# netease-youdao/EmotiVoice

Measured on NVIDIA H100. Metric: mel_frames_per_sec, higher is better.
Workload: dtype fp32 (fp32 storage + accumulate; tensor-core fp32 emulation: 3xTF32 prefix, bf16x3 after it)

## Files before the change

emotivoice_b200/csrc/conv1d_gp.cu:

```cuda
#include "ev_common.cuh"
#include "gp_pipeline.cuh"

namespace ev {
namespace gp {

using namespace gpl;

constexpr int MAX_A = 8;

struct GPlan {
  int BN, mt, kbg, planes;
  int rows_pad;
  int a_plane_bytes, b_plane_bytes, a_stage_bytes, b_stage_bytes;
  int a_stages, b_stages;
  int acc_cols;
  int tiles_m, tiles_n, total_tiles;
  int smem_total;
};

__host__ __device__ inline bool make_gplan(const GpConvParams& p, int mode, int BN, int mt, int kbg, GPlan* o, int span = -1, int kmin = 0, int ng = 1) {
  if (span < 0) span = (p.K - 1) * p.dil;
  if (kmin <= 0) kmin = p.K;
  GPlan q;
  q.planes = mode == 1 ? 2 : 1;
// ... 46 lines not shown
  __syncthreads();

  asm volatile("griddepcontrol.launch_dependents;" ::: "memory");

  const int n_cb = (p.Cin + KB - 1) / KB;
  const int tiles_per_b = pl.tiles_m * pl.tiles_n;
  const int tiles_per_g = p.B * tiles_per_b;

  auto decode = [&](int tile, int& gi, int& b, int& t0, int& n0, int& len) {
    gi = tile / tiles_per_g;
    tile -= gi * tiles_per_g;
    b = tile / tiles_per_b;
    const int r = tile - b * tiles_per_b;
    const int tm = r / pl.tiles_n, tn = r - tm * pl.tiles_n;
    t0 = tm * (BM * MT);
    n0 = tn * BN;
    len = p.lens ? min(p.L, p.lens[b] * p.lens_mul) : p.L;
  };

  if (warp < NCW) {
    asm volatile("griddepcontrol.wait;" ::: "memory");
    const int wg = warp >> 2, wl = warp & 3;
    const int coutR = p.Cout / p.rate;
    const int gout = coutR / CPG;
    const size_t Lout = (size_t)p.L * p.rate;
    const int accm = p.acc;
    const uint32_t a_lbo = (uint32_t)pl.rows_pad * 16u, b_lbo = (uint32_t)BN * 16u;
    const uint64_t a_desc0 = make_desc(0u, X3B ? 2u * a_lbo : a_lbo, 128u), b_desc0 = make_desc(0u, b_lbo, 128u);
    const uint32_t a_k8 = (X3B ? 4u : 2u) * a_lbo;
    const uint32_t a_lo_off = X3B ? a_lbo : (uint32_t)pl.a_plane_bytes;
    float acc[MT][NA];
#pragma unroll
    for (int mt = 0; mt < MT; ++mt)
#pragma unroll
      for (int i = 0; i < NA; ++i) acc[mt][i] = 0.f;
    int a_cnt = 0, b_cnt = 0;
    for (int tile = blockIdx.x; tile < pl.total_tiles; tile += gridDim.x) {
      int gi, b, t0, n0, len;
      decode(tile, gi, b, t0, n0, len);
      if (t0 >= len) continue;
      const GpGroup& G = gs.g[gi];
      const int K = G.K;
      const uint32_t a_tap = (uint32_t)G.dil * 16u;
      OneBehind<MAX_A> rel{ring, lane};
      for (int cb = 0; cb < n_cb; ++cb, ++a_cnt) {
        const int sa = a_cnt % pl.a_stages;
        const int nk8 = min(KB, p.Cin - cb * KB) / (2 * WCPG);
        mbar_wait(ring.a_ready(sa), (a_cnt / pl.a_stages) & 1);
        const uint64_t a_hi0 = desc_advance(a_desc0, smem_u32(a_tiles + sa * pl.a_stage_bytes) + (uint32_t)(wg * 64) * 16u);
        for (int j = 0; j < K; ++j, ++b_cnt) {
          const int sb = b_cnt % pl.b_stages;
          mbar_wait(ring.b_full(sb), (b_cnt / pl.b_stages) & 1);
          const uint64_t b_hi0 = desc_advance(b_desc0, smem_u32(b_tiles + sb * pl.b_stage_bytes));
          tap_chain<MODE, BN, NK8>(acc, desc_advance(a_hi0, (uint32_t)j * a_tap), a_k8, a_lo_off, b_hi0, (uint32_t)pl.b_plane_bytes, cb | j, nk8);
          wgmma_wait<1>();
          rel.step(sb, j == K - 1 ? sa : -1);
        }
      }

      constexpr int EQ = MT == 1 ? 2 : 1;
      const bool has_res = G.res != nullptr;
      const int row0 = t0 + wg * 64 + frag_row(0, lane, wl);
      float2 ebias[EQ];
      pair_t<BF16> eres[EQ][MT][2], eout[EQ][MT][2];
      auto column = [&](int q, int& n) {
        n = n0 + frag_col(4 * q, lane);
        const int phase = n / coutR, co = n - phase * coutR;
        return (((size_t)b * gout + co / CPG) * Lout + phase) * CPG + (co % CPG);
      };
      auto epi_load = [&](int ch) {
#pragma unroll
        for (int q = 0; q < EQ; ++q) {
          int n;
          const size_t ec = column(ch * EQ + q, n);
          if (n - n0 >= BN) continue;
          if (G.bias) ebias[q] = __ldg(reinterpret_cast<const float2*>(G.bias + n));
#pragma unroll
          for (int mt = 0; mt < MT; ++mt)
#pragma unroll
            for (int h = 0; h < 2; ++h) {
              const int row = row0 + mt * BM + 8 * h;
              if (row >= len) continue;
              const size_t e = ec + (size_t)row * p.rate * CPG;
              if (has_res) eres[q][mt][h] = load_pair<BF16>(G.res, e);
              if (accm != EV_ACC_STORE) eout[q][mt][h] = load_pair<BF16>(G.out, e);
            }
        }
      };
      auto epi_store = [&](int ch) {
#pragma unroll
        for (int q = 0; q < EQ; ++q) {
          int n;
          const size_t ec = column(ch * EQ + q, n);
          if (n - n0 >= BN) continue;
#pragma unroll
          for (int mt = 0; mt < MT; ++mt)
#pragma unroll
            for (int h = 0; h < 2; ++h) {
              const int row = row0 + mt * BM + 8 * h;
              if (row >= len) continue;
              const int i = 4 * (ch * EQ + q) + 2 * h;
              float v0 = acc[mt][i], v1 = acc[mt][i + 1];
              if (G.bias) { v0 += ebias[q].x; v1 += ebias[q].y; }
              if (has_res) {
                const float2 r = unpack_pair(eres[q][mt][h]);
                v0 += r.x; v1 += r.y;
              }
              if (accm != EV_ACC_STORE) {
// ... 457 lines not shown
```

emotivoice_b200/csrc/conv1d_tc.cu:

```cuda
#include <cstdio>
#include <cstdlib>

#include "ev_common.cuh"
#include "tc_common.cuh"

namespace ev {

namespace tc {

struct Plan {
  int BN, mt, kbg, planes;
  int rows_pad;
  int a_plane_bytes, b_plane_bytes, a_stage_bytes, b_stage_bytes;
  int a_stages, b_stages;
  int ngroups;
  int ksplit;
  int acc_cols;
  int tiles_m, tiles_n, total_tiles;
  int smem_total;
};

__host__ __device__ inline bool make_plan(const ConvParams& p, int mode, int BN, int mt, int kbg, int min_b_stages, Plan* o, int b_target = 4) {
  Plan q;
  q.planes = (mode == 1 || mode == 3) ? 2 : 1;
// ... 12 lines not shown
  const int budget = 227 * 1024 - 1024;
  const int n_cb = (p.Cin + cpg * q.kbg - 1) / (cpg * q.kbg);
  if (min_b_stages > n_cb * p.K) min_b_stages = n_cb * p.K;
  if (min_b_stages < 2) min_b_stages = 2;
  if (2 * q.a_stage_bytes + min_b_stages * q.b_stage_bytes > budget) return false;
  q.a_stages = 2;
  q.b_stages = 2;
  while (q.b_stages < MAX_B_STAGES && q.b_stages < n_cb * p.K &&
         q.a_stages * q.a_stage_bytes + (q.b_stages + 1) * q.b_stage_bytes <= budget && q.b_stages < b_target) ++q.b_stages;
  while (q.a_stages < MAX_A_STAGES && q.a_stages < n_cb &&
         (q.a_stages + 1) * q.a_stage_bytes + q.b_stages * q.b_stage_bytes <= budget && q.a_stages < 6) ++q.a_stages;
  while (q.b_stages < MAX_B_STAGES && q.b_stages < n_cb * p.K &&
         q.a_stages * q.a_stage_bytes + (q.b_stages + 1) * q.b_stage_bytes <= budget) ++q.b_stages;
  while (q.a_stages < MAX_A_STAGES && q.a_stages < n_cb &&
         (q.a_stages + 1) * q.a_stage_bytes + q.b_stages * q.b_stage_bytes <= budget) ++q.a_stages;
  q.ngroups = q.a_stages >= 6 ? 6 : (q.a_stages >= 3 ? 3 : (q.a_stages >= 2 ? 2 : 1));
  q.tiles_m = (p.L + BM * mt - 1) / (BM * mt);
  q.tiles_n = (p.Cout + q.BN - 1) / q.BN;
  q.ksplit = 1;
  q.total_tiles = p.B * q.tiles_m * q.tiles_n;
  q.smem_total = 1024 + q.a_stages * q.a_stage_bytes + q.b_stages * q.b_stage_bytes;
  *o = q;
  return true;
}

__device__ __forceinline__ void splitk_reduce_store(const ConvParams& p, int S, size_t per, size_t e, int b, int row, int col, int len) {
  float4 o = make_float4(0.f, 0.f, 0.f, 0.f);
  if (row < len) {
    for (int z = 0; z < S; ++z) {
      const float4 v = *reinterpret_cast<const float4*>(p.splitk_ws + (size_t)z * per + e);
      o.x += v.x; o.y += v.y; o.z += v.z; o.w += v.w;
    }
    if (p.bias) {
      const float4 b4 = __ldg(reinterpret_cast<const float4*>(p.bias + (size_t)b * p.bias_bs + col));
      o.x += b4.x; o.y += b4.y; o.z += b4.z; o.w += b4.w;
    }
    if (p.out_act != EV_ACT_NONE) {
      o.x = act_apply(o.x, p.out_act, 0.f); o.y = act_apply(o.y, p.out_act, 0.f);
      o.z = act_apply(o.z, p.out_act, 0.f); o.w = act_apply(o.w, p.out_act, 0.f);
    }
    if (p.res) {
      const float4 r4 = *reinterpret_cast<const float4*>(p.res + e);
      o.x += r4.x; o.y += r4.y; o.z += r4.z; o.w += r4.w;
    }
    if (p.acc != EV_ACC_STORE) {
      const float4 q4 = *reinterpret_cast<const float4*>(p.out + e);
      o.x += q4.x; o.y += q4.y; o.z += q4.z; o.w += q4.w;
      if (p.acc == EV_ACC_ADD_DIV) { o.x /= p.div; o.y /= p.div; o.z /= p.div; o.w /= p.div; }
    }
  }
  *reinterpret_cast<float4*>(p.out + e) = o;
}

template <int MODE, int MT, int KBG>
__global__ void __launch_bounds__(NTHREADS, 1) conv1d_tc_kernel(ConvParams p, Plan pl) {
  constexpr bool SPLIT3 = (MODE == 1);
  constexpr bool X3B = (MODE == 3);
  constexpr bool BF16 = (MODE == 2) || X3B;
  constexpr int PLANES = (SPLIT3 || X3B) ? 2 : 1;
  constexpr int CPG = BF16 ? 8 : 4;
  constexpr int KB = CPG * KBG;
  constexpr int GSH = (KBG == 8 ? 3 : 2);
  constexpr int NA = ACC_REGS / MT;
  constexpr int NCW = NCONS / 32;
  extern __shared__ __align__(128) uint8_t smem_raw[];
  const int tid = threadIdx.x;
  const int warp = __shfl_sync(0xffffffffu, tid >> 5, 0);
  const int lane = tid & 31;
  const int BN = pl.BN;

  uint64_t* bars = reinterpret_cast<uint64_t*>(smem_raw);
  uint8_t* a_tiles = smem_raw + 1024;
  uint8_t* b_tiles = a_tiles + pl.a_stages * pl.a_stage_bytes;
  const uint32_t bar_base = smem_u32(bars);
  auto a_full = [&](int s) { return bar_base + 8u * s; };
  auto a_empty = [&](int s) { return bar_base + 8u * (MAX_A_STAGES + s); };
  auto b_full = [&](int s) { return bar_base + 8u * (2 * MAX_A_STAGES + s); };
  auto b_empty = [&](int s) { return bar_base + 8u * (2 * MAX_A_STAGES + MAX_B_STAGES + s); };

  if (tid == 0) {
    for (int s = 0; s < pl.a_stages; ++s) { mbar_init(a_full(s), (NPWARPS / pl.ngroups) * 32); mbar_init(a_empty(s), NCW); }
    for (int s = 0; s < pl.b_stages; ++s) { mbar_init(b_full(s), 1); mbar_init(b_empty(s), NCW); }
    asm volatile("fence.mbarrier_init.release.cluster;" ::: "memory");
  }
  __syncthreads();

  asm volatile("griddepcontrol.launch_dependents;" ::: "memory");

  const int n_cb = (p.Cin + KB - 1) / KB;
  const int halo = ((p.K - 1) / 2) * p.dil;
  const int rows_a = BM * MT + (p.K - 1) * p.dil;
  const int tiles_per_b = pl.tiles_m * pl.tiles_n;

  int z_cur = 0;
  auto decode = [&](int tile, int& b, int& t0, int& n0, int& nt, int& len) {
    z_cur = tile % pl.ksplit;
    tile /= pl.ksplit;
    b = tile / tiles_per_b;
    const int r = tile - b * tiles_per_b;
    const int tm = r / pl.tiles_n, tn = r - tm * pl.tiles_n;
    t0 = tm * (BM * MT);
    n0 = tn * BN;
    nt = min(BN, p.Cout - n0);
    len = p.lens ? min(p.L, p.lens[b] * p.lens_mul) : p.L;
  };

  if (warp < NCW) {
    asm volatile("griddepcontrol.wait;" ::: "memory");
    const int wg = warp >> 2, wl = warp & 3;
    const bool split = pl.ksplit > 1;
    const bool has_res = p.res != nullptr && !split;
    const int oact = split ? EV_ACT_NONE : p.out_act, accm = split ? EV_ACC_STORE : p.acc;
    const uint32_t a_lbo = (uint32_t)pl.rows_pad * 16u, b_lbo = (uint32_t)BN * 16u;
    const uint64_t a_desc0 = make_desc(0u, a_lbo, 128u), b_desc0 = make_desc(0u, b_lbo, 128u);
    const uint32_t a_tap = (uint32_t)p.dil * 16u, a_k8 = 2u * a_lbo, b_k8 = 2u * b_lbo;
    float acc[MT][NA];
#pragma unroll
    for (int mt = 0; mt < MT; ++mt)
#pragma unroll
      for (int i = 0; i < NA; ++i) acc[mt][i] = 0.f;
    auto release = [&](int sb, int sa) {
      __syncwarp();
      if (lane == 0) {
        mbar_arrive(b_empty(sb));
        if (sa >= 0) mbar_arrive(a_empty(sa));
      }
    };
    int a_cnt = 0, b_cnt = 0;
    for (int tile = blockIdx.x; tile < pl.total_tiles; tile += gridDim.x) {
      int b, t0, n0, nt, len;
      decode(tile, b, t0, n0, nt, len);
      float* ob = (split ? p.splitk_ws + (size_t)z_cur * p.B * p.L * p.Cout : p.out) + (size_t)b * p.L * p.Cout;
      const float* rb = has_res ? p.res + (size_t)b * p.L * p.Cout : nullptr;
      const bool active = t0 < len;
      if (active) {
        const int cb_lo = (z_cur * n_cb) / pl.ksplit, cb_hi = ((z_cur + 1) * n_cb) / pl.ksplit;
        int prev_sb = -1, prev_sa = -1;
        for (int cb = cb_lo; cb < cb_hi; ++cb, ++a_cnt) {
          const int sa = a_cnt % pl.a_stages;
          const int nk8 = min(KB, p.Cin - cb * KB) / (2 * CPG);
          mbar_wait(a_full(sa), (a_cnt / pl.a_stages) & 1);
          const uint64_t a_hi0 = desc_advance(a_desc0, smem_u32(a_tiles + sa * pl.a_stage_bytes) + (uint32_t)(wg * 64) * 16u);
          for (int j = 0; j < p.K; ++j, ++b_cnt) {
            const int sb = b_cnt % pl.b_stages;
            mbar_wait(b_full(sb), (b_cnt / pl.b_stages) & 1);
            const uint64_t b_hi0 = desc_advance(b_desc0, smem_u32(b_tiles + sb * pl.b_stage_bytes));
            const uint64_t a_j = desc_advance(a_hi0, (uint32_t)j * a_tap);
            wgmma_fence();
            for (int k8 = 0; k8 < nk8; ++k8) {
              const uint64_t b_hi = desc_advance(b_hi0, (uint32_t)k8 * b_k8);
              const uint64_t b_lo = desc_advance(b_hi, (uint32_t)pl.b_plane_bytes);
              const uint64_t a_k = desc_advance(a_j, (uint32_t)k8 * a_k8);
              const uint32_t first = ((cb - cb_lo) | j | k8) != 0 ? 1u : 0u;
#pragma unroll
              for (int mt = 0; mt < MT; ++mt) {
                const uint64_t a_hi = desc_advance(a_k, (uint32_t)(mt * BM) * 16u);
                mma_step<MODE, NA>(nt, acc[mt], a_hi, desc_advance(a_hi, (uint32_t)pl.a_plane_bytes), b_hi, b_lo, first);
              }
            }
            wgmma_commit();
            wgmma_wait<1>();
            if (prev_sb >= 0) release(prev_sb, prev_sa);
            prev_sb = sb;
            prev_sa = j == p.K - 1 ? sa : -1;
          }
        }
        wgmma_wait<0>();
        release(prev_sb, prev_sa);
      }
      const float* __restrict__ bias = (p.bias && !split) ? p.bias + (size_t)b * p.bias_bs + n0 : nullptr;
#pragma unroll
      for (int mt = 0; mt < MT; ++mt) {
#pragma unroll
        for (int i = 0; i < NA; i += 2) {
          const int c = frag_col(i, lane);
          const int row = t0 + mt * BM + wg * 64 + frag_row(i, lane, wl);
          if (c >= nt || row >= p.L) continue;
          const size_t off = (size_t)row * p.Cout + n0 + c;
          float2 o = make_float2(0.f, 0.f);
          if (active && row < len) {
            o = make_float2(acc[mt][i], acc[mt][i + 1]);
            if (bias) {
              const float2 b2 = __ldg(reinterpret_cast<const float2*>(bias + c));
              o.x += b2.x; o.y += b2.y;
            }
            if (oact != EV_ACT_NONE) { o.x = act_apply(o.x, oact, 0.f); o.y = act_apply(o.y, oact, 0.f); }
            if (has_res) {
              const float2 r2 = *reinterpret_cast<const float2*>(rb + off);
              o.x += r2.x; o.y += r2.y;
            }
            if (accm != EV_ACC_STORE) {
              const float2 q2 = *reinterpret_cast<const float2*>(ob + off);
              o.x += q2.x; o.y += q2.y;
              if (accm == EV_ACC_ADD_DIV) { o.x /= p.div; o.y /= p.div; }
            }
          }
          *reinterpret_cast<float2*>(ob + off) = o;
        }
      }
    }
  } else if (warp < W_WLOAD) {
    asm volatile("griddepcontrol.wait;" ::: "memory");
    const int pwarp = warp - NCW;
    const int wpg = NPWARPS / pl.ngroups;
    const int grp = pwarp / wpg;
    const int gt = (pwarp - grp * wpg) * 32 + lane;
    const int GT = wpg * 32;
    const bool lrelu = (p.in_act == EV_ACT_LRELU);
    const float slope = p.in_slope;
    const int total = rows_a * KBG;
    int a_cnt = 0;
    for (int tile = blockIdx.x; tile < pl.total_tiles; tile += gridDim.x) {
      int b, t0, n0, nt, len;
      decode(tile, b, t0, n0, nt, len);
// ... 72 lines not shown
    if (lane == 0) {
      asm volatile("griddepcontrol.wait;" ::: "memory");
      const int cin4 = p.Cin / CPG;
      const int bnp = p.Cout < 128 ? p.Cout : 128;
      const size_t plane = (size_t)p.K * cin4 * p.Cout * 4;
      const size_t tile_stride = (size_t)p.K * cin4 * bnp * 4;
      int b_cnt = 0;
      for (int tile = blockIdx.x; tile < pl.total_tiles; tile += gridDim.x) {
        int b, t0, n0, nt, len;
        decode(tile, b, t0, n0, nt, len);
        if (t0 >= len) continue;
        const float* wt = p.w + (size_t)(n0 / bnp) * tile_stride + (size_t)(n0 % bnp) * 4;
        const int cb_lo = (z_cur * n_cb) / pl.ksplit, cb_hi = ((z_cur + 1) * n_cb) / pl.ksplit;
        for (int cb = cb_lo; cb < cb_hi; ++cb) {
          const int ngran = min(KB, p.Cin - cb * KB) / CPG;
          for (int j = 0; j < p.K; ++j, ++b_cnt) {
            const int sb = b_cnt % pl.b_stages;
            mbar_wait(b_empty(sb), ((b_cnt / pl.b_stages) & 1) ^ 1);
            mbar_expect_tx(b_full(sb), (uint32_t)(PLANES * ngran * nt * 16));
            const uint32_t dst = smem_u32(b_tiles + sb * pl.b_stage_bytes);
            const float* src = wt + ((size_t)j * cin4 + (size_t)cb * KBG) * bnp * 4;
            if (nt == bnp) {
              bulk_g2s(dst, src, (uint32_t)(ngran * nt * 16), b_full(sb));
              if (PLANES == 2) bulk_g2s(dst + (uint32_t)pl.b_plane_bytes, src + plane, (uint32_t)(ngran * nt * 16), b_full(sb));
            } else {
              for (int g = 0; g < ngran; ++g) {
                bulk_g2s(dst + (uint32_t)(g * BN * 16), src + (size_t)g * bnp * 4, (uint32_t)(nt * 16), b_full(sb));
                if (PLANES == 2) bulk_g2s(dst + (uint32_t)(pl.b_plane_bytes + g * BN * 16), src + plane + (size_t)g * bnp * 4, (uint32_t)(nt * 16), b_full(sb));
              }
            }
          }
        }
      }
    }
    __syncwarp();
  }
}

__global__ void __launch_bounds__(256) splitk_reduce_kernel(ConvParams p, int S) {
  pdl_entry();
  const size_t per = (size_t)p.B * p.L * p.Cout;
  const size_t i4 = (size_t)blockIdx.x * blockDim.x + threadIdx.x;
  if (i4 * 4 >= per) return;
  const size_t e = i4 * 4;
  const int col = (int)(e % p.Cout);
  const size_t rowg = e / p.Cout;
  const int b = (int)(rowg / p.L), row = (int)(rowg % p.L);
  const int len = p.lens ? min(p.L, p.lens[b] * p.lens_mul) : p.L;
  splitk_reduce_store(p, S, per, e, b, row, col, len);
}

}

template <int MODE, int MT, int KBG>
static int launch_tc_variant(const ConvParams& p, const tc::Plan& pl, cudaStream_t st) {
  static std::atomic<uint64_t> attr_devs{0};
  if (first_use_on_device(attr_devs))
    cudaFuncSetAttribute(tc::conv1d_tc_kernel<MODE, MT, KBG>, cudaFuncAttributeMaxDynamicSharedMemorySize, 227 * 1024);
  const int grid = pl.total_tiles < sm_count() ? pl.total_tiles : sm_count();
  return launch("conv1d_tc_kernel", tc::conv1d_tc_kernel<MODE, MT, KBG>, (unsigned)grid, tc::NTHREADS, pl.smem_total, st, p, pl);
}

template <int MODE, int KBG>
static int launch_tc_mt(const ConvParams& p, const tc::Plan& pl, cudaStream_t st) {
  if (pl.mt == 4) return launch_tc_variant<MODE, 4, KBG>(p, pl, st);
  if (pl.mt == 2) return launch_tc_variant<MODE, 2, KBG>(p, pl, st);
  return launch_tc_variant<MODE, 1, KBG>(p, pl, st);
}

template <int MODE, int KBG>
static void preload_tc_mode() {
  cudaFuncSetAttribute(tc::conv1d_tc_kernel<MODE, 1, KBG>, cudaFuncAttributeMaxDynamicSharedMemorySize, 227 * 1024);
  cudaFuncSetAttribute(tc::conv1d_tc_kernel<MODE, 2, KBG>, cudaFuncAttributeMaxDynamicSharedMemorySize, 227 * 1024);
  cudaFuncSetAttribute(tc::conv1d_tc_kernel<MODE, 4, KBG>, cudaFuncAttributeMaxDynamicSharedMemorySize, 227 * 1024);
}
void preload_conv1d_tc() {
  preload_tc_mode<0, 4>(); preload_tc_mode<0, 8>(); preload_tc_mode<1, 4>(); preload_tc_mode<2, 4>(); preload_tc_mode<2, 8>();
  preload_tc_mode<3, 4>(); preload_tc_mode<3, 8>();
  cudaFuncAttributes fa;
  cudaFuncGetAttributes(&fa, tc::splitk_reduce_kernel);
  cudaGetLastError();
}

static int validate_conv1d_tc(const ConvParams& p, int mode) {
  EV_CHECK_ARG(p.B > 0 && p.L > 0, "conv1d_tc: bad problem B=%d L=%d", p.B, p.L);
  EV_CHECK_ARG(p.Cin % (mode >= 2 ? 16 : 8) == 0, "conv1d_tc: Cin=%d must be a multiple of %d", p.Cin, mode >= 2 ? 16 : 8);
  EV_CHECK_ARG(p.Cout % 16 == 0 && (p.Cout <= 128 || p.Cout % 128 == 0), "conv1d_tc: Cout=%d must be a multiple of 16, and of 128 above 128", p.Cout);
  EV_CHECK_ARG(p.K >= 1 && (p.K & 1) && p.dil >= 1, "conv1d_tc: K=%d must be odd, dil=%d >= 1", p.K, p.dil);
  EV_CHECK_ARG(p.in_act == EV_ACT_NONE || p.in_act == EV_ACT_LRELU, "conv1d_tc: unsupported input activation");
  return EV_OK;
}

int tc_shape_kbg(const ConvParams& p, int mode) {
  tc::Plan pl;
  const int bn_max = p.Cout <= 128 ? p.Cout : 128;
  return (mode != 1 && tc::make_plan(p, mode, bn_max, 1, 8, 4, &pl)) ? 8 : 4;
}

static int apply_ksplit(const ConvParams& p, int mode, tc::Plan* pl) {
  const size_t per = (size_t)p.B * p.L * p.Cout;
  if (p.ksplit > 1 && (p.splitk_ws || p.splitk_cap == (size_t)-1)) {
    int S = p.ksplit;
    const int cpg = mode >= 2 ? 8 : 4;
    const int n_cb = (p.Cin + cpg * pl->kbg - 1) / (cpg * pl->kbg);
    if (S > n_cb) S = n_cb;
    if ((size_t)S * per > p.splitk_cap) { set_error("conv1d_tc: split-K scratch too small (%zu < %zu floats)", p.splitk_cap, (size_t)S * per); return EV_EWORKSPACE; }
    if (S > 1) {
      pl->ksplit = S;
      pl->total_tiles *= S;
    }
  }
  return EV_OK;
}

static int plan_conv1d_tc(const ConvParams& p, int mode, tc::Plan* out) {
  EV_TRY(validate_conv1d_tc(p, mode));
  const int bn_thresh = 24, mt_thresh = 120;
  const long long tiles128 = (long long)((p.L + tc::BM - 1) / tc::BM) * p.B;
  int BN = p.Cout <= 128 ? p.Cout : 128;
  while (BN >= 64 && (BN / 2) % 16 == 0 && tiles128 * ((p.Cout + BN - 1) / BN) < bn_thresh) BN /= 2;
  int mt = tiles128 >= 4 * mt_thresh ? 4 : (tiles128 >= 2 * mt_thresh ? 2 : 1);
  tc::Plan pl;
  const int kbg = tc_shape_kbg(p, mode);
  for (;; mt >>= 1) {
    if (tc::make_plan(p, mode, BN, mt, kbg, 4, &pl)) break;
    if (tc::make_plan(p, mode, BN, mt, kbg, 2, &pl)) break;
    if (mt == 1) { set_error("conv1d_tc: tile does not fit in shared memory / accumulator registers (K=%d dil=%d Cout=%d)", p.K, p.dil, p.Cout); return EV_EINVAL; }
  }
  EV_TRY(apply_ksplit(p, mode, &pl));
  *out = pl;
  return EV_OK;
}

int debug_tc_plan(const ConvParams& p, int mode, int* v) {
  tc::Plan pl;
  const int rc = plan_conv1d_tc(p, mode, &pl);
  if (rc != EV_OK) return rc;
  v[0] = pl.BN; v[1] = pl.mt; v[2] = pl.kbg; v[3] = pl.a_stages; v[4] = pl.b_stages; v[5] = pl.ngroups;
  v[6] = pl.ksplit; v[7] = pl.acc_cols; v[8] = pl.smem_total; v[9] = pl.total_tiles; v[10] = pl.rows_pad;
  return EV_OK;
}

static int dispatch_tc(const ConvParams& p, int mode, const tc::Plan& pl, cudaStream_t st) {
  if (mode == 1) return launch_tc_mt<1, 4>(p, pl, st);
  if (mode == 3) return pl.kbg == 8 ? launch_tc_mt<3, 8>(p, pl, st) : launch_tc_mt<3, 4>(p, pl, st);
  if (mode == 2) return pl.kbg == 8 ? launch_tc_mt<2, 8>(p, pl, st) : launch_tc_mt<2, 4>(p, pl, st);
  return pl.kbg == 8 ? launch_tc_mt<0, 8>(p, pl, st) : launch_tc_mt<0, 4>(p, pl, st);
}

int launch_conv1d_tc(const ConvParams& p, int mode, cudaStream_t st) {
  tc::Plan pl;
  EV_TRY(plan_conv1d_tc(p, mode, &pl));
  const size_t per = (size_t)p.B * p.L * p.Cout;
  const int rc = dispatch_tc(p, mode, pl, st);
  if (rc != EV_OK || pl.ksplit == 1) return rc;
  const size_t n4 = per / 4;
  return launch("splitk_reduce_kernel", tc::splitk_reduce_kernel, (unsigned)((n4 + 255) / 256), 256, 0, st, p, pl.ksplit);
}

}
```

emotivoice_b200/csrc/gp_pipeline.cuh:

```cuda
#pragma once
#include "tc_common.cuh"

namespace ev {
namespace gpl {

using namespace tc;

constexpr int NCW = 8;
constexpr int NTW = 4;
constexpr int W_XFORM = NCW;
constexpr int W_ALOAD = W_XFORM + NTW;
constexpr int W_BLOAD = W_ALOAD + 1;
constexpr int THREADS = (W_BLOAD + 1) * 32;
constexpr int MAX_B = 8;
constexpr int SMEM_HEAD = 1024;
constexpr int XF_UNROLL = 4;

__device__ __forceinline__ float lrelu_f(float v, float slope) { return fmaxf(v, v * slope); }

template <int MAX_A>
struct Ring {
  uint32_t base;
  __device__ __forceinline__ uint32_t a_full(int s) const { return base + 8u * s; }
  __device__ __forceinline__ uint32_t a_ready(int s) const { return base + 8u * (MAX_A + s); }
// ... 109 lines not shown
              v[u] = make_uint4(w4[0], w4[1], w4[2], w4[3]);
            }
            *reinterpret_cast<uint4*>(gb + r * 16) = v[u];
          } else {
            float4 t = make_float4(__uint_as_float(v[u].x), __uint_as_float(v[u].y), __uint_as_float(v[u].z), __uint_as_float(v[u].w));
            if (lrelu) { t.x = lrelu_f(t.x, slope); t.y = lrelu_f(t.y, slope); t.z = lrelu_f(t.z, slope); t.w = lrelu_f(t.w, slope); }
            const float4 h = make_float4(to_tf32(t.x), to_tf32(t.y), to_tf32(t.z), to_tf32(t.w));
            *reinterpret_cast<float4*>(gb + r * 16) = h;
            if (SPLIT3) {
              const float4 l = make_float4(to_tf32(t.x - h.x), to_tf32(t.y - h.y), to_tf32(t.z - h.z), to_tf32(t.w - h.w));
              *reinterpret_cast<float4*>(gb + plane_bytes + r * 16) = l;
            }
          }
        }
      }
    }
    fence_proxy_async();
    mbar_arrive(ring.a_ready(s));
  }
}

template <int MODE, int KBG, int N, int MAX_A>
__device__ __forceinline__ void load_w_tile(Ring<MAX_A> ring, int& b_cnt, int b_stages, uint8_t* b_tiles, int stage_bytes, int plane_bytes,
                                            const float* wt, int K, int Cin, int Cout, int bnp) {
  constexpr int PLANES = (MODE == 1 || MODE == 3) ? 2 : 1;
  constexpr int CPG = MODE == 2 ? 8 : 4;
  constexpr int WCPG = MODE >= 2 ? 8 : 4;
  constexpr int KB = CPG * KBG;
  constexpr int KBGW = KBG * CPG / WCPG;
  const int n_cb = (Cin + KB - 1) / KB;
  const int win = Cin / WCPG;
  const size_t plane = (size_t)K * win * Cout * 4;
  for (int cb = 0; cb < n_cb; ++cb) {
    const int ngran = min(KB, Cin - cb * KB) / WCPG;
    for (int j = 0; j < K; ++j, ++b_cnt) {
      const int sb = b_cnt % b_stages;
      mbar_wait(ring.b_empty(sb), ((b_cnt / b_stages) & 1) ^ 1);
      mbar_expect_tx(ring.b_full(sb), (uint32_t)(PLANES * ngran * N * 16));
      const uint32_t dst = smem_u32(b_tiles + sb * stage_bytes);
      const float* src = wt + ((size_t)j * win + (size_t)cb * KBGW) * bnp * 4;
      if (N == bnp) {
        bulk_g2s(dst, src, (uint32_t)(ngran * N * 16), ring.b_full(sb));
        if (PLANES == 2) bulk_g2s(dst + (uint32_t)plane_bytes, src + plane, (uint32_t)(ngran * N * 16), ring.b_full(sb));
      } else {
        for (int g = 0; g < ngran; ++g) {
          bulk_g2s(dst + (uint32_t)(g * N * 16), src + (size_t)g * bnp * 4, (uint32_t)(N * 16), ring.b_full(sb));
          if (PLANES == 2) bulk_g2s(dst + (uint32_t)(plane_bytes + g * N * 16), src + plane + (size_t)g * bnp * 4, (uint32_t)(N * 16), ring.b_full(sb));
        }
      }
    }
  }
}

template <int MODE, int N, int NK, int MT, int NA>
__device__ __forceinline__ void tap_chain(float (&acc)[MT][NA], uint64_t a, uint32_t a_step, uint32_t a_lo, uint64_t b, uint32_t b_lo, int cbj,
                                          int nk = NK) {
  auto k_step = [&](int k) {
    const uint64_t b_hi = desc_advance(b, (uint32_t)k * (2u * N * 16u));
    const uint64_t b_lo_k = desc_advance(b_hi, b_lo);
    const uint64_t a_k = desc_advance(a, (uint32_t)k * a_step);
    const uint32_t first = (cbj | k) != 0 ? 1u : 0u;
#pragma unroll
    for (int mt = 0; mt < MT; ++mt) {
      const uint64_t a_hi = desc_advance(a_k, (uint32_t)(mt * BM) * 16u);
      mma_step_fixed<MODE, N>(acc[mt], a_hi, desc_advance(a_hi, a_lo), b_hi, b_lo_k, first);
    }
  };
  wgmma_fence();
  if (nk == NK) {
#pragma unroll
    for (int k = 0; k < NK; ++k) k_step(k);
  } else {
#pragma unroll 1
    for (int k = 0; k < nk; ++k) k_step(k);
  }
  wgmma_commit();
}

template <int MAX_A>
struct OneBehind {
  Ring<MAX_A> ring;
  int lane;
  int sb = -1, sa = -1;
  __device__ __forceinline__ void release() const {
    __syncwarp();
    if (lane == 0) {
      mbar_arrive(ring.b_empty(sb));
      if (sa >= 0) mbar_arrive(ring.a_empty(sa));
    }
  }
  __device__ __forceinline__ void step(int sb_now, int sa_now) {
    if (sb >= 0) release();
    sb = sb_now;
    sa = sa_now;
  }
  __device__ __forceinline__ void drain() const { release(); }
};

}
}
```

emotivoice_b200/csrc/tc_common.cuh:

```cuda
#pragma once
#include <type_traits>
#include "ev_common.cuh"

namespace ev {
namespace tc {

constexpr int BM = 128;
constexpr int NCONS = 256;
constexpr int NPRODUCER = 192;
constexpr int W_WLOAD = (NCONS + NPRODUCER) / 32;
constexpr int NTHREADS = NCONS + NPRODUCER + 32;
constexpr int ACC_REGS = 64;
constexpr int A_LD = 8;
constexpr int MAX_A_STAGES = 8, MAX_B_STAGES = 8;
constexpr int NPWARPS = NPRODUCER / 32;

__device__ __forceinline__ uint32_t smem_u32(const void* p) { return (uint32_t)__cvta_generic_to_shared(p); }

__device__ __forceinline__ void mbar_init(uint32_t bar, uint32_t count) {
  asm volatile("mbarrier.init.shared::cta.b64 [%0], %1;" ::"r"(bar), "r"(count));
}
__device__ __forceinline__ void mbar_arrive(uint32_t bar) {
  asm volatile("mbarrier.arrive.shared::cta.b64 _, [%0];" ::"r"(bar) : "memory");
}
// ... 105 lines not shown
               "wgmma.mma_async.sync.aligned.m64n128k8.f32.tf32.tf32 {%0,%1,%2,%3,%4,%5,%6,%7,%8,%9,%10,%11,%12,%13,%14,%15,%16,%17,%18,%19,%20,%21,%22,%23,%24,%25,%26,%27,%28,%29,%30,%31,%32,%33,%34,%35,%36,%37,%38,%39,%40,%41,%42,%43,%44,%45,%46,%47,%48,%49,%50,%51,%52,%53,%54,%55,%56,%57,%58,%59,%60,%61,%62,%63}, %64, %65, p, 1, 1;\n\t}"
               : "+f"(d[0]), "+f"(d[1]), "+f"(d[2]), "+f"(d[3]), "+f"(d[4]), "+f"(d[5]), "+f"(d[6]), "+f"(d[7]), "+f"(d[8]), "+f"(d[9]), "+f"(d[10]), "+f"(d[11]), "+f"(d[12]), "+f"(d[13]), "+f"(d[14]), "+f"(d[15]), "+f"(d[16]), "+f"(d[17]), "+f"(d[18]), "+f"(d[19]), "+f"(d[20]), "+f"(d[21]), "+f"(d[22]), "+f"(d[23]), "+f"(d[24]), "+f"(d[25]), "+f"(d[26]), "+f"(d[27]), "+f"(d[28]), "+f"(d[29]), "+f"(d[30]), "+f"(d[31]), "+f"(d[32]), "+f"(d[33]), "+f"(d[34]), "+f"(d[35]), "+f"(d[36]), "+f"(d[37]), "+f"(d[38]), "+f"(d[39]), "+f"(d[40]), "+f"(d[41]), "+f"(d[42]), "+f"(d[43]), "+f"(d[44]), "+f"(d[45]), "+f"(d[46]), "+f"(d[47]), "+f"(d[48]), "+f"(d[49]), "+f"(d[50]), "+f"(d[51]), "+f"(d[52]), "+f"(d[53]), "+f"(d[54]), "+f"(d[55]), "+f"(d[56]), "+f"(d[57]), "+f"(d[58]), "+f"(d[59]), "+f"(d[60]), "+f"(d[61]), "+f"(d[62]), "+f"(d[63])
               : "l"(a), "l"(b), "r"(acc));
}
__device__ __forceinline__ void wgmma_bf16_n16(float* d, uint64_t a, uint64_t b, uint32_t acc) {
  asm volatile("{\n\t.reg .pred p;\n\tsetp.ne.b32 p, %10, 0;\n\t"
               "wgmma.mma_async.sync.aligned.m64n16k16.f32.bf16.bf16 {%0,%1,%2,%3,%4,%5,%6,%7}, %8, %9, p, 1, 1, 0, 0;\n\t}"
               : "+f"(d[0]), "+f"(d[1]), "+f"(d[2]), "+f"(d[3]), "+f"(d[4]), "+f"(d[5]), "+f"(d[6]), "+f"(d[7])
               : "l"(a), "l"(b), "r"(acc));
}
__device__ __forceinline__ void wgmma_bf16_n32(float* d, uint64_t a, uint64_t b, uint32_t acc) {
  asm volatile("{\n\t.reg .pred p;\n\tsetp.ne.b32 p, %18, 0;\n\t"
               "wgmma.mma_async.sync.aligned.m64n32k16.f32.bf16.bf16 {%0,%1,%2,%3,%4,%5,%6,%7,%8,%9,%10,%11,%12,%13,%14,%15}, %16, %17, p, 1, 1, 0, 0;\n\t}"
               : "+f"(d[0]), "+f"(d[1]), "+f"(d[2]), "+f"(d[3]), "+f"(d[4]), "+f"(d[5]), "+f"(d[6]), "+f"(d[7]), "+f"(d[8]), "+f"(d[9]), "+f"(d[10]), "+f"(d[11]), "+f"(d[12]), "+f"(d[13]), "+f"(d[14]), "+f"(d[15])
               : "l"(a), "l"(b), "r"(acc));
}
__device__ __forceinline__ void wgmma_bf16_n48(float* d, uint64_t a, uint64_t b, uint32_t acc) {
  asm volatile("{\n\t.reg .pred p;\n\tsetp.ne.b32 p, %26, 0;\n\t"
               "wgmma.mma_async.sync.aligned.m64n48k16.f32.bf16.bf16 {%0,%1,%2,%3,%4,%5,%6,%7,%8,%9,%10,%11,%12,%13,%14,%15,%16,%17,%18,%19,%20,%21,%22,%23}, %24, %25, p, 1, 1, 0, 0;\n\t}"
               : "+f"(d[0]), "+f"(d[1]), "+f"(d[2]), "+f"(d[3]), "+f"(d[4]), "+f"(d[5]), "+f"(d[6]), "+f"(d[7]), "+f"(d[8]), "+f"(d[9]), "+f"(d[10]), "+f"(d[11]), "+f"(d[12]), "+f"(d[13]), "+f"(d[14]), "+f"(d[15]), "+f"(d[16]), "+f"(d[17]), "+f"(d[18]), "+f"(d[19]), "+f"(d[20]), "+f"(d[21]), "+f"(d[22]), "+f"(d[23])
               : "l"(a), "l"(b), "r"(acc));
}
__device__ __forceinline__ void wgmma_bf16_n64(float* d, uint64_t a, uint64_t b, uint32_t acc) {
  asm volatile("{\n\t.reg .pred p;\n\tsetp.ne.b32 p, %34, 0;\n\t"
               "wgmma.mma_async.sync.aligned.m64n64k16.f32.bf16.bf16 {%0,%1,%2,%3,%4,%5,%6,%7,%8,%9,%10,%11,%12,%13,%14,%15,%16,%17,%18,%19,%20,%21,%22,%23,%24,%25,%26,%27,%28,%29,%30,%31}, %32, %33, p, 1, 1, 0, 0;\n\t}"
               : "+f"(d[0]), "+f"(d[1]), "+f"(d[2]), "+f"(d[3]), "+f"(d[4]), "+f"(d[5]), "+f"(d[6]), "+f"(d[7]), "+f"(d[8]), "+f"(d[9]), "+f"(d[10]), "+f"(d[11]), "+f"(d[12]), "+f"(d[13]), "+f"(d[14]), "+f"(d[15]), "+f"(d[16]), "+f"(d[17]), "+f"(d[18]), "+f"(d[19]), "+f"(d[20]), "+f"(d[21]), "+f"(d[22]), "+f"(d[23]), "+f"(d[24]), "+f"(d[25]), "+f"(d[26]), "+f"(d[27]), "+f"(d[28]), "+f"(d[29]), "+f"(d[30]), "+f"(d[31])
               : "l"(a), "l"(b), "r"(acc));
}
__device__ __forceinline__ void wgmma_bf16_n80(float* d, uint64_t a, uint64_t b, uint32_t acc) {
  asm volatile("{\n\t.reg .pred p;\n\tsetp.ne.b32 p, %42, 0;\n\t"
               "wgmma.mma_async.sync.aligned.m64n80k16.f32.bf16.bf16 {%0,%1,%2,%3,%4,%5,%6,%7,%8,%9,%10,%11,%12,%13,%14,%15,%16,%17,%18,%19,%20,%21,%22,%23,%24,%25,%26,%27,%28,%29,%30,%31,%32,%33,%34,%35,%36,%37,%38,%39}, %40, %41, p, 1, 1, 0, 0;\n\t}"
               : "+f"(d[0]), "+f"(d[1]), "+f"(d[2]), "+f"(d[3]), "+f"(d[4]), "+f"(d[5]), "+f"(d[6]), "+f"(d[7]), "+f"(d[8]), "+f"(d[9]), "+f"(d[10]), "+f"(d[11]), "+f"(d[12]), "+f"(d[13]), "+f"(d[14]), "+f"(d[15]), "+f"(d[16]), "+f"(d[17]), "+f"(d[18]), "+f"(d[19]), "+f"(d[20]), "+f"(d[21]), "+f"(d[22]), "+f"(d[23]), "+f"(d[24]), "+f"(d[25]), "+f"(d[26]), "+f"(d[27]), "+f"(d[28]), "+f"(d[29]), "+f"(d[30]), "+f"(d[31]), "+f"(d[32]), "+f"(d[33]), "+f"(d[34]), "+f"(d[35]), "+f"(d[36]), "+f"(d[37]), "+f"(d[38]), "+f"(d[39])
               : "l"(a), "l"(b), "r"(acc));
}
__device__ __forceinline__ void wgmma_bf16_n96(float* d, uint64_t a, uint64_t b, uint32_t acc) {
  asm volatile("{\n\t.reg .pred p;\n\tsetp.ne.b32 p, %50, 0;\n\t"
               "wgmma.mma_async.sync.aligned.m64n96k16.f32.bf16.bf16 {%0,%1,%2,%3,%4,%5,%6,%7,%8,%9,%10,%11,%12,%13,%14,%15,%16,%17,%18,%19,%20,%21,%22,%23,%24,%25,%26,%27,%28,%29,%30,%31,%32,%33,%34,%35,%36,%37,%38,%39,%40,%41,%42,%43,%44,%45,%46,%47}, %48, %49, p, 1, 1, 0, 0;\n\t}"
               : "+f"(d[0]), "+f"(d[1]), "+f"(d[2]), "+f"(d[3]), "+f"(d[4]), "+f"(d[5]), "+f"(d[6]), "+f"(d[7]), "+f"(d[8]), "+f"(d[9]), "+f"(d[10]), "+f"(d[11]), "+f"(d[12]), "+f"(d[13]), "+f"(d[14]), "+f"(d[15]), "+f"(d[16]), "+f"(d[17]), "+f"(d[18]), "+f"(d[19]), "+f"(d[20]), "+f"(d[21]), "+f"(d[22]), "+f"(d[23]), "+f"(d[24]), "+f"(d[25]), "+f"(d[26]), "+f"(d[27]), "+f"(d[28]), "+f"(d[29]), "+f"(d[30]), "+f"(d[31]), "+f"(d[32]), "+f"(d[33]), "+f"(d[34]), "+f"(d[35]), "+f"(d[36]), "+f"(d[37]), "+f"(d[38]), "+f"(d[39]), "+f"(d[40]), "+f"(d[41]), "+f"(d[42]), "+f"(d[43]), "+f"(d[44]), "+f"(d[45]), "+f"(d[46]), "+f"(d[47])
               : "l"(a), "l"(b), "r"(acc));
}
__device__ __forceinline__ void wgmma_bf16_n112(float* d, uint64_t a, uint64_t b, uint32_t acc) {
  asm volatile("{\n\t.reg .pred p;\n\tsetp.ne.b32 p, %58, 0;\n\t"
               "wgmma.mma_async.sync.aligned.m64n112k16.f32.bf16.bf16 {%0,%1,%2,%3,%4,%5,%6,%7,%8,%9,%10,%11,%12,%13,%14,%15,%16,%17,%18,%19,%20,%21,%22,%23,%24,%25,%26,%27,%28,%29,%30,%31,%32,%33,%34,%35,%36,%37,%38,%39,%40,%41,%42,%43,%44,%45,%46,%47,%48,%49,%50,%51,%52,%53,%54,%55}, %56, %57, p, 1, 1, 0, 0;\n\t}"
               : "+f"(d[0]), "+f"(d[1]), "+f"(d[2]), "+f"(d[3]), "+f"(d[4]), "+f"(d[5]), "+f"(d[6]), "+f"(d[7]), "+f"(d[8]), "+f"(d[9]), "+f"(d[10]), "+f"(d[11]), "+f"(d[12]), "+f"(d[13]), "+f"(d[14]), "+f"(d[15]), "+f"(d[16]), "+f"(d[17]), "+f"(d[18]), "+f"(d[19]), "+f"(d[20]), "+f"(d[21]), "+f"(d[22]), "+f"(d[23]), "+f"(d[24]), "+f"(d[25]), "+f"(d[26]), "+f"(d[27]), "+f"(d[28]), "+f"(d[29]), "+f"(d[30]), "+f"(d[31]), "+f"(d[32]), "+f"(d[33]), "+f"(d[34]), "+f"(d[35]), "+f"(d[36]), "+f"(d[37]), "+f"(d[38]), "+f"(d[39]), "+f"(d[40]), "+f"(d[41]), "+f"(d[42]), "+f"(d[43]), "+f"(d[44]), "+f"(d[45]), "+f"(d[46]), "+f"(d[47]), "+f"(d[48]), "+f"(d[49]), "+f"(d[50]), "+f"(d[51]), "+f"(d[52]), "+f"(d[53]), "+f"(d[54]), "+f"(d[55])
               : "l"(a), "l"(b), "r"(acc));
}
__device__ __forceinline__ void wgmma_bf16_n128(float* d, uint64_t a, uint64_t b, uint32_t acc) {
  asm volatile("{\n\t.reg .pred p;\n\tsetp.ne.b32 p, %66, 0;\n\t"
               "wgmma.mma_async.sync.aligned.m64n128k16.f32.bf16.bf16 {%0,%1,%2,%3,%4,%5,%6,%7,%8,%9,%10,%11,%12,%13,%14,%15,%16,%17,%18,%19,%20,%21,%22,%23,%24,%25,%26,%27,%28,%29,%30,%31,%32,%33,%34,%35,%36,%37,%38,%39,%40,%41,%42,%43,%44,%45,%46,%47,%48,%49,%50,%51,%52,%53,%54,%55,%56,%57,%58,%59,%60,%61,%62,%63}, %64, %65, p, 1, 1, 0, 0;\n\t}"
               : "+f"(d[0]), "+f"(d[1]), "+f"(d[2]), "+f"(d[3]), "+f"(d[4]), "+f"(d[5]), "+f"(d[6]), "+f"(d[7]), "+f"(d[8]), "+f"(d[9]), "+f"(d[10]), "+f"(d[11]), "+f"(d[12]), "+f"(d[13]), "+f"(d[14]), "+f"(d[15]), "+f"(d[16]), "+f"(d[17]), "+f"(d[18]), "+f"(d[19]), "+f"(d[20]), "+f"(d[21]), "+f"(d[22]), "+f"(d[23]), "+f"(d[24]), "+f"(d[25]), "+f"(d[26]), "+f"(d[27]), "+f"(d[28]), "+f"(d[29]), "+f"(d[30]), "+f"(d[31]), "+f"(d[32]), "+f"(d[33]), "+f"(d[34]), "+f"(d[35]), "+f"(d[36]), "+f"(d[37]), "+f"(d[38]), "+f"(d[39]), "+f"(d[40]), "+f"(d[41]), "+f"(d[42]), "+f"(d[43]), "+f"(d[44]), "+f"(d[45]), "+f"(d[46]), "+f"(d[47]), "+f"(d[48]), "+f"(d[49]), "+f"(d[50]), "+f"(d[51]), "+f"(d[52]), "+f"(d[53]), "+f"(d[54]), "+f"(d[55]), "+f"(d[56]), "+f"(d[57]), "+f"(d[58]), "+f"(d[59]), "+f"(d[60]), "+f"(d[61]), "+f"(d[62]), "+f"(d[63])
               : "l"(a), "l"(b), "r"(acc));
}

template <bool BF16, int NA>
__device__ __forceinline__ void wgmma_n(int n, float (&d)[NA], uint64_t a, uint64_t b, uint32_t acc) {
#define EV_WG_CASE(N)                                                    \
  case N:                                                                \
    if constexpr (2 * NA >= N) {                                         \
      if (BF16) wgmma_bf16_n##N(d, a, b, acc); else wgmma_tf32_n##N(d, a, b, acc); \
    }                                                                    \
    break;
  switch (n) {
    EV_WG_CASE(16) EV_WG_CASE(32) EV_WG_CASE(48) EV_WG_CASE(64) EV_WG_CASE(80) EV_WG_CASE(96) EV_WG_CASE(112) EV_WG_CASE(128)
    default: break;
  }
#undef EV_WG_CASE
}

template <bool BF16, int N, int NA>
__device__ __forceinline__ void wgmma_fixed(float (&d)[NA], uint64_t a, uint64_t b, uint32_t acc) {
  static_assert(N % 32 == 0 && N <= 128 && N <= 2 * NA, "N tile must be 32 / 64 / 96 / 128 and fit the accumulator");
  if constexpr (N == 32) { if constexpr (BF16) wgmma_bf16_n32(d, a, b, acc); else wgmma_tf32_n32(d, a, b, acc); }
  else if constexpr (N == 64) { if constexpr (BF16) wgmma_bf16_n64(d, a, b, acc); else wgmma_tf32_n64(d, a, b, acc); }
  else if constexpr (N == 96) { if constexpr (BF16) wgmma_bf16_n96(d, a, b, acc); else wgmma_tf32_n96(d, a, b, acc); }
  else { if constexpr (BF16) wgmma_bf16_n128(d, a, b, acc); else wgmma_tf32_n128(d, a, b, acc); }
}

template <int MODE, int NA>
__device__ __forceinline__ void mma_step(int n, float (&d)[NA], uint64_t a_hi, uint64_t a_lo, uint64_t b_hi, uint64_t b_lo, uint32_t acc) {
  constexpr bool OP16 = MODE >= 2;
  if (MODE == 1 || MODE == 3) {
    wgmma_n<OP16, NA>(n, d, a_lo, b_hi, acc);
    wgmma_n<OP16, NA>(n, d, a_hi, b_lo, 1u);
    wgmma_n<OP16, NA>(n, d, a_hi, b_hi, 1u);
  } else {
    wgmma_n<OP16, NA>(n, d, a_hi, b_hi, acc);
  }
}

template <int MODE, int N, int NA>
__device__ __forceinline__ void mma_step_fixed(float (&d)[NA], uint64_t a_hi, uint64_t a_lo, uint64_t b_hi, uint64_t b_lo, uint32_t acc) {
  constexpr bool OP16 = MODE >= 2;
  if constexpr (MODE == 1 || MODE == 3) {
    wgmma_fixed<OP16, N>(d, a_lo, b_hi, acc);
    wgmma_fixed<OP16, N>(d, a_hi, b_lo, 1u);
    wgmma_fixed<OP16, N>(d, a_hi, b_hi, 1u);
  } else {
    wgmma_fixed<OP16, N>(d, a_hi, b_hi, acc);
  }
}

}
}
```

Baseline: 109,900.

## Specialize conv1d tensor-core kernel on compile-time N tile width

```diff
diff --git a/emotivoice_b200/csrc/conv1d_gp.cu b/emotivoice_b200/csrc/conv1d_gp.cu
--- a/emotivoice_b200/csrc/conv1d_gp.cu
+++ b/emotivoice_b200/csrc/conv1d_gp.cu
@@ -122,8 +122,14 @@
           const int sb = b_cnt % pl.b_stages;
           mbar_wait(ring.b_full(sb), (b_cnt / pl.b_stages) & 1);
           const uint64_t b_hi0 = desc_advance(b_desc0, smem_u32(b_tiles + sb * pl.b_stage_bytes));
-          tap_chain<MODE, BN, NK8>(acc, desc_advance(a_hi0, (uint32_t)j * a_tap), a_k8, a_lo_off, b_hi0, (uint32_t)pl.b_plane_bytes, cb | j, nk8);
-          wgmma_wait<1>();
+          const uint64_t a_j = desc_advance(a_hi0, (uint32_t)j * a_tap);
+          if (nk8 == NK8) {
+            tap_chain<MODE, BN, NK8>(acc, a_j, a_k8, a_lo_off, b_hi0, (uint32_t)pl.b_plane_bytes, cb | j);
+            wgmma_wait<1>();
+          } else {
+            tap_chain_short<MODE, BN>(acc, a_j, a_k8, a_lo_off, b_hi0, (uint32_t)pl.b_plane_bytes, cb | j, nk8);
+            wgmma_wait<1>();
+          }
           rel.step(sb, j == K - 1 ? sa : -1);
         }
       }
diff --git a/emotivoice_b200/csrc/conv1d_tc.cu b/emotivoice_b200/csrc/conv1d_tc.cu
--- a/emotivoice_b200/csrc/conv1d_tc.cu
+++ b/emotivoice_b200/csrc/conv1d_tc.cu
@@ -88,7 +88,7 @@
   *reinterpret_cast<float4*>(p.out + e) = o;
 }
 
-template <int MODE, int MT, int KBG>
+template <int MODE, int MT, int KBG, int BN>
 __global__ void __launch_bounds__(NTHREADS, 1) conv1d_tc_kernel(ConvParams p, Plan pl) {
   constexpr bool SPLIT3 = (MODE == 1);
   constexpr bool X3B = (MODE == 3);
@@ -96,14 +96,15 @@
   constexpr int PLANES = (SPLIT3 || X3B) ? 2 : 1;
   constexpr int CPG = BF16 ? 8 : 4;
   constexpr int KB = CPG * KBG;
+  constexpr int NK8 = KBG / 2;
   constexpr int GSH = (KBG == 8 ? 3 : 2);
-  constexpr int NA = ACC_REGS / MT;
+  constexpr int NA = BN / 2;
   constexpr int NCW = NCONS / 32;
+  static_assert(BN % 16 == 0 && MT * BN <= 2 * ACC_REGS, "accumulators of the tile exceed the register budget");
   extern __shared__ __align__(128) uint8_t smem_raw[];
   const int tid = threadIdx.x;
   const int warp = __shfl_sync(0xffffffffu, tid >> 5, 0);
   const int lane = tid & 31;
-  const int BN = pl.BN;
 
   uint64_t* bars = reinterpret_cast<uint64_t*>(smem_raw);
   uint8_t* a_tiles = smem_raw + 1024;
@@ -149,7 +150,7 @@
     const int oact = split ? EV_ACT_NONE : p.out_act, accm = split ? EV_ACC_STORE : p.acc;
     const uint32_t a_lbo = (uint32_t)pl.rows_pad * 16u, b_lbo = (uint32_t)BN * 16u;
     const uint64_t a_desc0 = make_desc(0u, a_lbo, 128u), b_desc0 = make_desc(0u, b_lbo, 128u);
-    const uint32_t a_tap = (uint32_t)p.dil * 16u, a_k8 = 2u * a_lbo, b_k8 = 2u * b_lbo;
+    const uint32_t a_tap = (uint32_t)p.dil * 16u, a_k8 = 2u * a_lbo;
     float acc[MT][NA];
 #pragma unroll
     for (int mt = 0; mt < MT; ++mt)
@@ -182,20 +183,13 @@
             mbar_wait(b_full(sb), (b_cnt / pl.b_stages) & 1);
             const uint64_t b_hi0 = desc_advance(b_desc0, smem_u32(b_tiles + sb * pl.b_stage_bytes));
             const uint64_t a_j = desc_advance(a_hi0, (uint32_t)j * a_tap);
-            wgmma_fence();
-            for (int k8 = 0; k8 < nk8; ++k8) {
-              const uint64_t b_hi = desc_advance(b_hi0, (uint32_t)k8 * b_k8);
-              const uint64_t b_lo = desc_advance(b_hi, (uint32_t)pl.b_plane_bytes);
-              const uint64_t a_k = desc_advance(a_j, (uint32_t)k8 * a_k8);
-              const uint32_t first = ((cb - cb_lo) | j | k8) != 0 ? 1u : 0u;
-#pragma unroll
-              for (int mt = 0; mt < MT; ++mt) {
-                const uint64_t a_hi = desc_advance(a_k, (uint32_t)(mt * BM) * 16u);
-                mma_step<MODE, NA>(nt, acc[mt], a_hi, desc_advance(a_hi, (uint32_t)pl.a_plane_bytes), b_hi, b_lo, first);
-              }
-            }
-            wgmma_commit();
-            wgmma_wait<1>();
+            if (nk8 == NK8) {
+              tap_chain<MODE, BN, NK8>(acc, a_j, a_k8, (uint32_t)pl.a_plane_bytes, b_hi0, (uint32_t)pl.b_plane_bytes, (cb - cb_lo) | j);
+              wgmma_wait<1>();
+            } else {
+              tap_chain_short<MODE, BN>(acc, a_j, a_k8, (uint32_t)pl.a_plane_bytes, b_hi0, (uint32_t)pl.b_plane_bytes, (cb - cb_lo) | j, nk8);
+              wgmma_wait<1>();
+            }
             if (prev_sb >= 0) release(prev_sb, prev_sa);
             prev_sb = sb;
             prev_sa = j == p.K - 1 ? sa : -1;
@@ -374,31 +368,37 @@
 
 }
 
-template <int MODE, int MT, int KBG>
-static int launch_tc_variant(const ConvParams& p, const tc::Plan& pl, cudaStream_t st) {
-  static std::atomic<uint64_t> attr_devs{0};
-  if (first_use_on_device(attr_devs))
-    cudaFuncSetAttribute(tc::conv1d_tc_kernel<MODE, MT, KBG>, cudaFuncAttributeMaxDynamicSharedMemorySize, 227 * 1024);
-  const int grid = pl.total_tiles < sm_count() ? pl.total_tiles : sm_count();
-  return launch("conv1d_tc_kernel", tc::conv1d_tc_kernel<MODE, MT, KBG>, (unsigned)grid, tc::NTHREADS, pl.smem_total, st, p, pl);
-}
-
+using TcKernel = void (*)(ConvParams, tc::Plan);
 template <int MODE, int KBG>
-static int launch_tc_mt(const ConvParams& p, const tc::Plan& pl, cudaStream_t st) {
-  if (pl.mt == 4) return launch_tc_variant<MODE, 4, KBG>(p, pl, st);
-  if (pl.mt == 2) return launch_tc_variant<MODE, 2, KBG>(p, pl, st);
-  return launch_tc_variant<MODE, 1, KBG>(p, pl, st);
-}
-
-template <int MODE, int KBG>
-static void preload_tc_mode() {
-  cudaFuncSetAttribute(tc::conv1d_tc_kernel<MODE, 1, KBG>, cudaFuncAttributeMaxDynamicSharedMemorySize, 227 * 1024);
-  cudaFuncSetAttribute(tc::conv1d_tc_kernel<MODE, 2, KBG>, cudaFuncAttributeMaxDynamicSharedMemorySize, 227 * 1024);
-  cudaFuncSetAttribute(tc::conv1d_tc_kernel<MODE, 4, KBG>, cudaFuncAttributeMaxDynamicSharedMemorySize, 227 * 1024);
-}
+static TcKernel tc_kernel_tile(int mt, int bn) {
+  using namespace tc;
+  switch (bn) {
+    case 128: return mt == 1 ? conv1d_tc_kernel<MODE, 1, KBG, 128> : nullptr;
+    case 112: return mt == 1 ? conv1d_tc_kernel<MODE, 1, KBG, 112> : nullptr;
+    case 96: return mt == 1 ? conv1d_tc_kernel<MODE, 1, KBG, 96> : nullptr;
+    case 80: return mt == 1 ? conv1d_tc_kernel<MODE, 1, KBG, 80> : nullptr;
+    case 64: return mt == 2 ? conv1d_tc_kernel<MODE, 2, KBG, 64> : mt == 1 ? conv1d_tc_kernel<MODE, 1, KBG, 64> : nullptr;
+    case 48: return mt == 2 ? conv1d_tc_kernel<MODE, 2, KBG, 48> : mt == 1 ? conv1d_tc_kernel<MODE, 1, KBG, 48> : nullptr;
+    case 32: return mt == 4 ? conv1d_tc_kernel<MODE, 4, KBG, 32> : mt == 2 ? conv1d_tc_kernel<MODE, 2, KBG, 32>
+                  : mt == 1 ? conv1d_tc_kernel<MODE, 1, KBG, 32> : nullptr;
+    case 16: return mt == 4 ? conv1d_tc_kernel<MODE, 4, KBG, 16> : mt == 2 ? conv1d_tc_kernel<MODE, 2, KBG, 16>
+                  : mt == 1 ? conv1d_tc_kernel<MODE, 1, KBG, 16> : nullptr;
+    default: return nullptr;
+  }
+}
+static TcKernel tc_kernel(int mode, int kbg, int mt, int bn) {
+  if (mode == 1) return kbg == 4 ? tc_kernel_tile<1, 4>(mt, bn) : nullptr;
+  if (mode == 3) return kbg == 8 ? tc_kernel_tile<3, 8>(mt, bn) : tc_kernel_tile<3, 4>(mt, bn);
+  if (mode == 2) return kbg == 8 ? tc_kernel_tile<2, 8>(mt, bn) : tc_kernel_tile<2, 4>(mt, bn);
+  return kbg == 8 ? tc_kernel_tile<0, 8>(mt, bn) : tc_kernel_tile<0, 4>(mt, bn);
+}
+
 void preload_conv1d_tc() {
-  preload_tc_mode<0, 4>(); preload_tc_mode<0, 8>(); preload_tc_mode<1, 4>(); preload_tc_mode<2, 4>(); preload_tc_mode<2, 8>();
-  preload_tc_mode<3, 4>(); preload_tc_mode<3, 8>();
+  for (int mode = 0; mode < 4; ++mode)
+    for (int kbg = 4; kbg <= 8; kbg += 4)
+      for (int bn = 16; bn <= 128; bn += 16)
+        for (int mt = 1; mt <= 4 && mt * bn <= 128; mt *= 2)
+          if (const TcKernel k = tc_kernel(mode, kbg, mt, bn)) cudaFuncSetAttribute(k, cudaFuncAttributeMaxDynamicSharedMemorySize, 227 * 1024);
   cudaFuncAttributes fa;
   cudaFuncGetAttributes(&fa, tc::splitk_reduce_kernel);
   cudaGetLastError();
@@ -464,10 +464,12 @@
 }
 
 static int dispatch_tc(const ConvParams& p, int mode, const tc::Plan& pl, cudaStream_t st) {
-  if (mode == 1) return launch_tc_mt<1, 4>(p, pl, st);
-  if (mode == 3) return pl.kbg == 8 ? launch_tc_mt<3, 8>(p, pl, st) : launch_tc_mt<3, 4>(p, pl, st);
-  if (mode == 2) return pl.kbg == 8 ? launch_tc_mt<2, 8>(p, pl, st) : launch_tc_mt<2, 4>(p, pl, st);
-  return pl.kbg == 8 ? launch_tc_mt<0, 8>(p, pl, st) : launch_tc_mt<0, 4>(p, pl, st);
+  static std::atomic<uint64_t> attr_devs{0};
+  if (first_use_on_device(attr_devs)) preload_conv1d_tc();
+  const TcKernel k = tc_kernel(mode, pl.kbg, pl.mt, pl.BN);
+  EV_CHECK_ARG(k, "conv1d_tc: no kernel for mode %d, KBG %d, MT %d, BN %d", mode, pl.kbg, pl.mt, pl.BN);
+  const int grid = pl.total_tiles < sm_count() ? pl.total_tiles : sm_count();
+  return launch("conv1d_tc_kernel", k, (unsigned)grid, tc::NTHREADS, pl.smem_total, st, p, pl);
 }
 
 int launch_conv1d_tc(const ConvParams& p, int mode, cudaStream_t st) {
diff --git a/emotivoice_b200/csrc/gp_pipeline.cuh b/emotivoice_b200/csrc/gp_pipeline.cuh
--- a/emotivoice_b200/csrc/gp_pipeline.cuh
+++ b/emotivoice_b200/csrc/gp_pipeline.cuh
@@ -185,31 +185,6 @@
   }
 }
 
-template <int MODE, int N, int NK, int MT, int NA>
-__device__ __forceinline__ void tap_chain(float (&acc)[MT][NA], uint64_t a, uint32_t a_step, uint32_t a_lo, uint64_t b, uint32_t b_lo, int cbj,
-                                          int nk = NK) {
-  auto k_step = [&](int k) {
-    const uint64_t b_hi = desc_advance(b, (uint32_t)k * (2u * N * 16u));
-    const uint64_t b_lo_k = desc_advance(b_hi, b_lo);
-    const uint64_t a_k = desc_advance(a, (uint32_t)k * a_step);
-    const uint32_t first = (cbj | k) != 0 ? 1u : 0u;
-#pragma unroll
-    for (int mt = 0; mt < MT; ++mt) {
-      const uint64_t a_hi = desc_advance(a_k, (uint32_t)(mt * BM) * 16u);
-      mma_step_fixed<MODE, N>(acc[mt], a_hi, desc_advance(a_hi, a_lo), b_hi, b_lo_k, first);
-    }
-  };
-  wgmma_fence();
-  if (nk == NK) {
-#pragma unroll
-    for (int k = 0; k < NK; ++k) k_step(k);
-  } else {
-#pragma unroll 1
-    for (int k = 0; k < nk; ++k) k_step(k);
-  }
-  wgmma_commit();
-}
-
 template <int MAX_A>
 struct OneBehind {
   Ring<MAX_A> ring;
diff --git a/emotivoice_b200/csrc/tc_common.cuh b/emotivoice_b200/csrc/tc_common.cuh
--- a/emotivoice_b200/csrc/tc_common.cuh
+++ b/emotivoice_b200/csrc/tc_common.cuh
@@ -181,40 +181,17 @@
                : "l"(a), "l"(b), "r"(acc));
 }
 
-template <bool BF16, int NA>
-__device__ __forceinline__ void wgmma_n(int n, float (&d)[NA], uint64_t a, uint64_t b, uint32_t acc) {
-#define EV_WG_CASE(N)                                                    \
-  case N:                                                                \
-    if constexpr (2 * NA >= N) {                                         \
-      if (BF16) wgmma_bf16_n##N(d, a, b, acc); else wgmma_tf32_n##N(d, a, b, acc); \
-    }                                                                    \
-    break;
-  switch (n) {
-    EV_WG_CASE(16) EV_WG_CASE(32) EV_WG_CASE(48) EV_WG_CASE(64) EV_WG_CASE(80) EV_WG_CASE(96) EV_WG_CASE(112) EV_WG_CASE(128)
-    default: break;
-  }
-#undef EV_WG_CASE
-}
-
 template <bool BF16, int N, int NA>
 __device__ __forceinline__ void wgmma_fixed(float (&d)[NA], uint64_t a, uint64_t b, uint32_t acc) {
-  static_assert(N % 32 == 0 && N <= 128 && N <= 2 * NA, "N tile must be 32 / 64 / 96 / 128 and fit the accumulator");
-  if constexpr (N == 32) { if constexpr (BF16) wgmma_bf16_n32(d, a, b, acc); else wgmma_tf32_n32(d, a, b, acc); }
+  static_assert(N % 16 == 0 && N >= 16 && N <= 128 && N <= 2 * NA, "N tile must be a multiple of 16 up to 128 and fit the accumulator");
+  if constexpr (N == 16) { if constexpr (BF16) wgmma_bf16_n16(d, a, b, acc); else wgmma_tf32_n16(d, a, b, acc); }
+  else if constexpr (N == 32) { if constexpr (BF16) wgmma_bf16_n32(d, a, b, acc); else wgmma_tf32_n32(d, a, b, acc); }
+  else if constexpr (N == 48) { if constexpr (BF16) wgmma_bf16_n48(d, a, b, acc); else wgmma_tf32_n48(d, a, b, acc); }
   else if constexpr (N == 64) { if constexpr (BF16) wgmma_bf16_n64(d, a, b, acc); else wgmma_tf32_n64(d, a, b, acc); }
+  else if constexpr (N == 80) { if constexpr (BF16) wgmma_bf16_n80(d, a, b, acc); else wgmma_tf32_n80(d, a, b, acc); }
   else if constexpr (N == 96) { if constexpr (BF16) wgmma_bf16_n96(d, a, b, acc); else wgmma_tf32_n96(d, a, b, acc); }
+  else if constexpr (N == 112) { if constexpr (BF16) wgmma_bf16_n112(d, a, b, acc); else wgmma_tf32_n112(d, a, b, acc); }
   else { if constexpr (BF16) wgmma_bf16_n128(d, a, b, acc); else wgmma_tf32_n128(d, a, b, acc); }
-}
-
-template <int MODE, int NA>
-__device__ __forceinline__ void mma_step(int n, float (&d)[NA], uint64_t a_hi, uint64_t a_lo, uint64_t b_hi, uint64_t b_lo, uint32_t acc) {
-  constexpr bool OP16 = MODE >= 2;
-  if (MODE == 1 || MODE == 3) {
-    wgmma_n<OP16, NA>(n, d, a_lo, b_hi, acc);
-    wgmma_n<OP16, NA>(n, d, a_hi, b_lo, 1u);
-    wgmma_n<OP16, NA>(n, d, a_hi, b_hi, 1u);
-  } else {
-    wgmma_n<OP16, NA>(n, d, a_hi, b_hi, acc);
-  }
 }
 
 template <int MODE, int N, int NA>
@@ -229,5 +206,38 @@
   }
 }
 
-}
-}
+template <int MODE, int N, int MT, int NA>
+__device__ __forceinline__ void tap_k_step(float (&acc)[MT][NA], uint64_t a, uint32_t a_step, uint32_t a_lo, uint64_t b, uint32_t b_lo,
+                                           int cbj, int k) {
+  const uint64_t b_hi = desc_advance(b, (uint32_t)k * (2u * N * 16u));
+  const uint64_t b_lo_k = desc_advance(b_hi, b_lo);
+  const uint64_t a_k = desc_advance(a, (uint32_t)k * a_step);
+  const uint32_t first = (cbj | k) != 0 ? 1u : 0u;
+#pragma unroll
+  for (int mt = 0; mt < MT; ++mt) {
+    const uint64_t a_hi = desc_advance(a_k, (uint32_t)(mt * BM) * 16u);
+    mma_step_fixed<MODE, N>(acc[mt], a_hi, desc_advance(a_hi, a_lo), b_hi, b_lo_k, first);
+  }
+}
+
+template <int MODE, int N, int NK, int MT, int NA>
+__device__ __forceinline__ void tap_chain(float (&acc)[MT][NA], uint64_t a, uint32_t a_step, uint32_t a_lo, uint64_t b, uint32_t b_lo, int cbj) {
+  wgmma_fence();
+#pragma unroll
+  for (int k = 0; k < NK; ++k) tap_k_step<MODE, N>(acc, a, a_step, a_lo, b, b_lo, cbj, k);
+  wgmma_commit();
+}
+
+template <int MODE, int N, int MT, int NA>
+__device__ __forceinline__ void tap_chain_short(float (&acc)[MT][NA], uint64_t a, uint32_t a_step, uint32_t a_lo, uint64_t b, uint32_t b_lo,
+                                                int cbj, int nk) {
+#pragma unroll 1
+  for (int k = 0; k < nk; ++k) {
+    wgmma_fence();
+    tap_k_step<MODE, N>(acc, a, a_step, a_lo, b, b_lo, cbj, k);
+  }
+  wgmma_commit();
+}
+
+}
+}
```

After: 121,100, median of 6. 1.1x the previous value.
